# EStormLynn/Peter-Shirley-Ray-Tracing-the-next-week

Hardware: AMD Instinct MI355X
Metric: Msamples/s (pixels×spp/s) + achieved HBM GB/s, final() 500×500×1000spp (higher is better)
Workload: dtype f32

## Files before the change

### include/rt_hip.h

```cpp
#ifndef RT_HIP_H
#define RT_HIP_H
#include <stdint.h>

#ifdef __cplusplus
extern "C" {
#endif

#define RT_ABI_VERSION 2

typedef enum rt_status {
    RT_OK = 0,
    RT_ERR_INVALID = -1,
    RT_ERR_HIP = -2,
    RT_ERR_NOMEM = -3,
    RT_ERR_UNSUPPORTED = -4
} rt_status;

enum rt_prim_kind {
    RT_PRIM_SPHERE = 0,
    RT_PRIM_MOVING_SPHERE = 1,
    RT_PRIM_XY_RECT = 2,
    RT_PRIM_XZ_RECT = 3,
    RT_PRIM_YZ_RECT = 4
};

typedef struct rt_prim {
    int32_t kind;
    int32_t material;
    int32_t instance;
    int32_t flip;
    float p[12];
// ... 123 lines not shown
    double cycles_media;
    double cycles_shade;
    double grid;
    double wave_iterations;
    double wave_node_trips;
    double wave_prim_trips;
    double wave_sphere_draw_trips;
    double lane_sphere_draw_trips;
    double chunk;
    double batches;
    double lds_level;
    double stack_depth;
    double scan_groups;
    double prescan;
    double wave_exhaust_first_us;
    double wave_exhaust_last_us;
    double wave_end_first_us;
    double wave_end_mean_us;
    double wave_end_last_us;
    double wave_shade_passes;
    double wave_shade_kinds;
    double lane_scatters;
    double cycles_scatter;
} rt_stats;

typedef struct rt_scene rt_scene;

int rt_scene_create(const rt_scene_desc *d, int device, rt_scene **out);
void rt_scene_destroy(rt_scene *s);

int rt_render_tile(rt_scene *s, const rt_camera_desc *cam, const rt_render_params *p,
                   int x0, int y0, int w, int h, float *out_rgb, rt_stats *stats);

int rt_render_tiles(rt_scene *s, const rt_camera_desc *cam, const rt_render_params *p,
                    const int32_t *tiles, int ntiles, float *out_dev, void *stream, rt_stats *stats);

int rt_device_alloc(int device, uint64_t bytes, void **out);
int rt_device_free(void *ptr);
int rt_copy_to_host(void *dst, const void *src_dev, uint64_t bytes);
int rt_device_count(int *out);

int rt_math_probe(int fn, const float *a, const float *b, float *out, int64_t n);

#define RT_DIST_ID_BYTES 128
typedef struct rt_dist rt_dist;
int rt_dist_unique_id(uint8_t id[RT_DIST_ID_BYTES]);
// ... 45 lines not shown
```

### peter-shirley-ray-tracing-the-next-week_amd/csrc/hip/rt_device.h

```cpp
#pragma once
#include <hip/hip_runtime.h>
#include <stdint.h>
#include <type_traits>

#include "rt_layout.h"
#include "rt_libm.h"
#include "rt_log_table.h"
#include "rt_kernel.h"

#define RT_FLT_MAX 0x1.fffffep+127f
#ifndef RT_SHADE_LEAN
#define RT_SHADE_LEAN 117
#endif
#define RT_INF __builtin_huge_valf()

namespace {

__device__ __forceinline__ uint64_t wballot(bool b) { return __builtin_amdgcn_ballot_w64(b); }

struct V3 { float x, y, z; };
__device__ __forceinline__ V3 mk(float a, float b, float c) { V3 r; r.x = a; r.y = b; r.z = c; return r; }
__device__ __forceinline__ float unset_f() {
    float x;
    asm volatile("; unset %0" : "=v"(x));
    return x;
}
__device__ __forceinline__ V3 unset_v3() { return mk(unset_f(), unset_f(), unset_f()); }
__device__ __forceinline__ V3 add(V3 a, V3 b) { return mk(a.x + b.x, a.y + b.y, a.z + b.z); }
__device__ __forceinline__ V3 sub(V3 a, V3 b) { return mk(a.x - b.x, a.y - b.y, a.z - b.z); }
__device__ __forceinline__ V3 mul(V3 a, V3 b) { return mk(a.x * b.x, a.y * b.y, a.z * b.z); }
__device__ __forceinline__ V3 scale(float t, V3 v) { return mk(t * v.x, t * v.y, t * v.z); }
__device__ __forceinline__ V3 divs(V3 v, float t) { return mk(v.x / t, v.y / t, v.z / t); }
__device__ __forceinline__ V3 neg(V3 v) { return mk(-v.x, -v.y, -v.z); }
__device__ __forceinline__ float dot(V3 a, V3 b) { return a.x * b.x + a.y * b.y + a.z * b.z; }
__device__ __forceinline__ float len(V3 v) { return sqrtf(v.x * v.x + v.y * v.y + v.z * v.z); }
__device__ __forceinline__ V3 unit(V3 v) { return divs(v, len(v)); }
__device__ __forceinline__ float comp(V3 v, int i) { return i == 0 ? v.x : (i == 1 ? v.y : v.z); }

struct Ray { V3 o, d; float time; };

__device__ __forceinline__ float div_rn(float x, float b, float y) {
    const float q = x * y;
    return __builtin_fmaf(__builtin_fmaf(-q, b, x), y, q);
}
__device__ __forceinline__ V3 divs_rn(V3 v, float t, float y) { return mk(div_rn(v.x, t, y), div_rn(v.y, t, y), div_rn(v.z, t, y)); }
__device__ __forceinline__ bool normal_recip(float y) {
    const float m = __builtin_fabsf(y);
    return m >= 0x1p-126f && m <= 0x1.fffffep+127f;
}
struct Recip { float a, y; bool ok; };
__device__ __forceinline__ Recip recip_of(float a, bool use) {
    Recip r;
    r.a = a;
    r.y = 1.0f / a;
    r.ok = wballot(use && !normal_recip(r.y)) == 0ull;
    return r;
}
__device__ __forceinline__ float div_by(float x, const Recip &r) { return r.ok ? div_rn(x, r.a, r.y) : x / r.a; }
__device__ __forceinline__ V3 at(const Ray &r, float t) { return add(r.o, scale(t, r.d)); }

constexpr uint64_t kGamma = 0x9E3779B97F4A7C15ull;
constexpr uint64_t kLcgA = 0x5DEECE66Dull, kLcgC = 0xBull, kLcgM = 0xFFFFFFFFFFFFull;
__host__ __device__ __forceinline__ uint64_t mix64(uint64_t z) {
    z = (z ^ (z >> 30)) * 0xBF58476D1CE4E5B9ull;
    z = (z ^ (z >> 27)) * 0x94D049BB133111EBull;
    return z ^ (z >> 31);
}
__device__ __forceinline__ double u48(uint64_t z) {
    const uint64_t bits = 0x3FF0000000000000ull | ((z >> 12) & 0x000FFFFFFFFFFFF0ull);
    return __longlong_as_double((long long)bits) - 1.0;
}
__device__ __forceinline__ double u48x(uint64_t x) {
    return __longlong_as_double((long long)(0x3FF0000000000000ull | (x << 4))) - 1.0;
}
__device__ __forceinline__ uint64_t lcg_step(uint64_t x) {
    const uint32_t xl = (uint32_t)x, xh = (uint32_t)(x >> 32);
    static_assert(kLcgC == 11, "the drand48 increment is the inline constant of v_mad_u64_u32 below");
    uint64_t p, cy;
    uint32_t hi;
    asm("v_mad_u64_u32 %0, %1, %2, %3, 11" : "=v"(p), "=s"(cy) : "v"(xl), "s"(0xDEECE66Du));
    asm("v_mad_u32_u16 %0, %1, 5, %2" : "=v"(hi) : "v"(xl), "v"((uint32_t)(p >> 32)));
    asm("v_mad_u32_u16 %0, %1, %2, %3" : "=v"(hi) : "v"(xh), "s"(0xE66Du), "v"(hi));
    return ((uint64_t)(hi & 0xFFFFu) << 32) | (uint32_t)p;
}
typedef unsigned U4j __attribute__((ext_vector_type(4)));
__device__ __forceinline__ uint64_t lcg_jump(uint64_t x, U4j jt) {
    const uint32_t xl = (uint32_t)x, xh = (uint32_t)(x >> 32);
    const uint64_t c = ((uint64_t)jt.w << 32) | jt.z;
    uint64_t p, cy;
    uint32_t hi;
    asm("v_mad_u64_u32 %0, %1, %2, %3, %4" : "=v"(p), "=s"(cy) : "v"(xl), "v"(jt.x), "v"(c));
    asm("v_mad_u32_u16 %0, %1, %2, %3" : "=v"(hi) : "v"(xl), "v"(jt.y), "v"((uint32_t)(p >> 32)));
    asm("v_mad_u32_u16 %0, %1, %2, %3" : "=v"(hi) : "v"(xh), "v"(jt.x), "v"(hi));
    return ((uint64_t)(hi & 0xFFFFu) << 32) | (uint32_t)p;
}
#define RT_LCG_JUMPS 193
// ... 258 lines not shown
            float oi, di, oj, dj;
            if (kind == RT_PRIM_XY_RECT) { oi = r.o.x; di = r.d.x; oj = r.o.y; dj = r.d.y; }
            else if (kind == RT_PRIM_XZ_RECT) { oi = r.o.x; di = r.d.x; oj = r.o.z; dj = r.d.z; }
            else { oi = r.o.y; di = r.d.y; oj = r.o.z; dj = r.d.z; }
            const float a = oi + t * di, b = oj + t * dj;
            h.u = (a - g0.x) / (g0.y - g0.x);
            h.v = (b - g0.z) / (g0.w - g0.z);
        }
    }
    if (flip) h.n = neg(h.n);
    if (kInst && inst >= 0) to_world(insts, inst, h.p, h.n);
    return h;
}

__device__ __forceinline__ uint32_t lanes_below(uint64_t mask);
__device__ __forceinline__ bool first_active() { return lanes_below(wballot(1)) == 0; }

struct Counters {
    uint64_t samples = 0, segments = 0, nodes = 0, spheres = 0, mspheres = 0, rects = 0, instanced = 0, media = 0,
             shades = 0, noise = 0;
    uint64_t w_iters = 0, w_nodes = 0, w_prims = 0, w_rius = 0, l_rius = 0;
    uint64_t w_shade = 0, w_kinds = 0, l_scatter = 0;
    uint64_t ball[RT_BALL_N] = {0, 0, 0, 0, 0, 0, 0, 0};
    __device__ __forceinline__ void prim(int kind) {
        const int k = kind & 0xff;
        if (k == RT_PRIM_SPHERE) spheres++;
        else if (k == RT_PRIM_MOVING_SPHERE) mspheres++;
        else rects++;
        if (kind & 0x100) instanced++;
    }
};

template <bool kCount, bool kInst = true>
__device__ __forceinline__ float boundary_t(const float4 *B, const float4 *insts, int first, int count, const Ray &r,
                                            float tmin, Counters &cnt) {
    float best = RT_INF;
    for (int q = 0; q < count; ++q) {
        int key, kind;
        float t = prim_t<kInst>(B, insts, (uint32_t)(first + q), r, tmin, key, kind);
        if (kCount) cnt.prim(kind);
        if (t < best) best = t;
    }
    return best;
}

template <class RV, class PM>
// ... 626 lines not shown
}

typedef LogConsts MediaConsts;
typedef __attribute__((address_space(3))) const volatile MediaConsts LdsMediaConsts;
struct MediumRec {
    int4 md;
    float4 g0;
    float4 mm;
};
#ifndef RT_LDS_MEDIA
#define RT_LDS_MEDIA 8
#endif
template <int kBlock>
__device__ __forceinline__ void load_media(const RtKernelArgs &A, MediumRec *lds) {
    const int n = min(A.nmedia, RT_LDS_MEDIA);
    for (int i = threadIdx.x; i < n; i += kBlock) {
        const int4 md = A.media[i];
        lds[i].md = md;
        lds[i].g0 = A.bprims[md.x * 4 + 0];
        lds[i].mm = A.bprims[md.x * 4 + 1];
    }
}

template <bool kCount, bool kInst = true>
__device__ __forceinline__ void medium_one(const RtKernelArgs &A, const MediumRec &M, int k, const Ray &r, const Recip &rd,
                                           const Recip &ra, uint64_t xk, bool &have, float &best_t,
                                           int &med_mat, LdsMediaConsts *mc, Counters &cnt) {
    const float dlen = rd.a;
    if (kCount) cnt.media++;
    const int4 md = M.md;
    float r1, r2;
    bool ok;
    const float4 bm = M.mm;
    if (md.y == 1 && (fbits(bm.x) & 0xff) == RT_PRIM_SPHERE && fbits(bm.z) < 0) {
        if (kCount) cnt.spheres++;
        const float4 sg = M.g0;
        V3 oc = sub(r.o, mk(sg.x, sg.y, sg.z));
        const float a = ra.a;
        float b = dot(oc, r.d);
        float cc = dot(oc, oc) - sg.w * sg.w;
        float disc = b * b - a * cc;
        const bool valid = disc > 0;
        if (wballot(valid) == 0ull) return;
        const float sq = sqrtf(disc);
        const float ta = div_by(-b - sq, ra);
        const float tb = div_by(-b + sq, ra);
        const bool fa = ta < RT_FLT_MAX && ta > -RT_FLT_MAX, fb = tb < RT_FLT_MAX && tb > -RT_FLT_MAX;
        r1 = fa ? ta : tb;
        const float tmin2 = (float)((double)r1 + 0.0001);
        const bool ga = ta < RT_FLT_MAX && ta > tmin2, gb = tb < RT_FLT_MAX && tb > tmin2;
        r2 = ga ? ta : tb;
        ok = valid && (fa || fb) && (ga || gb);
    } else {
        r1 = boundary_t<kCount, kInst>(A.bprims, A.insts, md.x, md.y, r, -RT_FLT_MAX, cnt);
        ok = r1 != RT_INF;
        if (wballot(ok) == 0ull) return;
        r2 = boundary_t<kCount, kInst>(A.bprims, A.insts, md.x, md.y, r, (float)((double)r1 + 0.0001), cnt);
        ok = ok && r2 != RT_INF;
    }
    const float tmax = have ? best_t : RT_FLT_MAX;
    r1 = r1 < A.tmin ? A.tmin : r1;
    r2 = r2 > tmax ? tmax : r2;
    ok = ok && !(r1 >= r2);
    if (wballot(ok) == 0ull) return;
    r1 = r1 < 0 ? 0.f : r1;
    const float distance_inside_boundary = (r2 - r1) * dlen;
    const float neg_inv_density = __int_as_float(md.z);
#if !defined(__HIP_DEVICE_COMPILE__)
    const LogConsts lc{mc->c07, mc->c06, mc->c02, mc->c025, mc->c03};
#else
    uint32_t mca = (uint32_t)(size_t)mc;
    asm volatile("" : "+v"(mca));
    const LogConsts lc = *(__attribute__((address_space(3))) const LogConsts *)(size_t)mca;
#endif
    const float hit_distance = (float)((double)neg_inv_density * log_f64(u48x(xk), lc));
    const bool hit = ok && hit_distance < distance_inside_boundary;
    const float tm = r1 + div_by(hit_distance, rd);
    best_t = hit ? tm : best_t;
    have = have || hit;
    med_mat = hit ? md.w : med_mat;
}

template <bool kCount, bool kInst = true>
__device__ __forceinline__ int media_hit(const RtKernelArgs &A, const MediumRec *lds_media, LdsMediaConsts *mc, const Ray &r,
                                         const Recip &rd, Rng &g, bool &have, float &best_t, Counters &cnt) {
    const Recip ra = recip_of(dot(r.d, r.d), true);
    typedef unsigned U4v __attribute__((ext_vector_type(4)));
    typedef __attribute__((address_space(3))) const U4v LdsU4;
    int med_mat = -1;
    const int nl = min(A.nmedia, RT_LDS_MEDIA);
    for (int k = 0; k < nl; ++k) {
        const LdsU4 *p = (const LdsU4 *)lds_media + 3 * k;
        const U4v x = p[0], y = p[1], z = p[2];
        MediumRec M;
        M.md = make_int4((int)x.x, (int)x.y, (int)x.z, (int)x.w);
        M.g0 = make_float4(__uint_as_float(y.x), __uint_as_float(y.y), __uint_as_float(y.z), __uint_as_float(y.w));
        M.mm = make_float4(__uint_as_float(z.x), __uint_as_float(z.y), __uint_as_float(z.z), __uint_as_float(z.w));
        g.xm = lcg_step(g.xm);
        medium_one<kCount, kInst>(A, M, k, r, rd, ra, g.xm, have, best_t, med_mat, mc, cnt);
    }
    for (int k = RT_LDS_MEDIA; k < A.nmedia; ++k) {
        MediumRec M;
        M.md = A.media[k];
        M.g0 = A.bprims[M.md.x * 4 + 0];
        M.mm = A.bprims[M.md.x * 4 + 1];
        g.xm = lcg_step(g.xm);
        medium_one<kCount, kInst>(A, M, k, r, rd, ra, g.xm, have, best_t, med_mat, mc, cnt);
    }
    return med_mat;
}

struct ShadeOut {
    bool scattered;
    V3 att, emitted;
    Ray ray;
};

struct ShadeState {
    int kind;
    bool live;
    bool wants_sphere;
    V3 tv;
};

template <bool kCount, bool kUV = true, bool kChecker = true, class RV = const float4 *, class PM = const int *>
__device__ __forceinline__ ShadeState shade_begin(const RtKernelArgs &A, bool ready, bool have, const Hit &hr, int depth,
                                                  CoopSlot *slots, uint32_t lane, Counters &cnt, RV ranvec, PM perm) {
    const bool shading = ready && have;
    ShadeState st;
    st.kind = -1;
    st.live = false;
// ... 124 lines not shown
```

### peter-shirley-ray-tracing-the-next-week_amd/csrc/hip/rt_kernel.h

```cpp
#pragma once
#include <hip/hip_runtime.h>
#include <stdint.h>

#define RT_BLOCK 256

#define RT_LDS_BLOCK 1024
#define RT_LDS_NODE_CAP 1024
#define RT_LDS_NODE_BYTES (4 * RT_LDS_NODE_CAP * 16)
#define RT_LDS_NODE_BYTES_MEDIA (14 * RT_LDS_NODE_CAP * 4)
#define RT_LDS_STACK_BYTES(depth) ((RT_LDS_BLOCK / 64) * (depth) * 64 * 2)
#define RT_LDS_MAX_PRIMS 4096
#define RT_LDS_BUDGET 163840

#define RT_FEAT_INST 1
#define RT_FEAT_UV 2
#define RT_FEAT_CHECKER 4
#define RT_FEAT_PRESCAN 8
#define RT_FEAT_MEDIA 16
#define RT_FEAT_ALL 31

#define RT_WAVE_LOG_WORDS 12

struct RtKernelArgs {
    const float4 *nodes;
// ... 6 lines not shown
    const float4 *ranvec;
    const int *perm;
    const uint8_t *texels;
    uint32_t root;
    uint32_t nnodes;
    int bvh_width;
    int has_bvh;
    int nmedia;
    int features;
    int need_dlen;
    const float4 *groups;
    int ngroups;
    int scan;
    uint32_t nprims;
    int nprescan;
    int cell_first, cell_n;
    float cell_c[3], cell_r2;
    float cell_rin2;
    int ball_waves;
    int ball_batch;
    int ball_claim;
    int ball_park;
    int ball_drain;
    int lds_nodes;
    int stack_depth;
    float org[3], llc[3], hor[3], ver[3], cu[3], cv[3];
    float lens, ct0, ct1;
    int nx, ny, ns, max_depth;
    float rnx, rny;
    float tmin;
    int background;
    int chunk, nchunks;
    uint32_t sample_offset;
    uint64_t seed;
    const uint32_t *job_xy;
    uint32_t npix;
    uint32_t nitems;
    uint32_t ndeep;
    uint32_t ndeep_items;
    uint32_t claim;
    uint32_t nbig;
    uint32_t claim_tail;
    float *slab;
    uint32_t *counter;
    unsigned long long *stats;
    unsigned long long *wave_log;
// ... 16 lines not shown
```

### peter-shirley-ray-tracing-the-next-week_amd/csrc/hip/rt_kernel.hip

```cpp
#include <algorithm>
#include <atomic>
#include <type_traits>

#include "rt_device.h"

namespace {


#define RT_SLAB_FLOATS 3
#ifndef RT_READY_BATCH
#define RT_READY_BATCH 48
#endif

#ifndef RT_DESCEND_STEPS
#define RT_DESCEND_STEPS 2
#endif


#ifndef RT_DRY_LANES
#define RT_DRY_LANES 16
#endif


#define RT_PRE 64
// ... 507 lines not shown
                            if (wballot(ra || rb) == 0ull) test_pair(std::integral_constant<int, 1>());
                            else if (wballot(!ra || sb) == 0ull) test_pair(std::integral_constant<int, 2>());
                            else test_pair(std::integral_constant<int, 3>());
                        }
                    }
                    if (node == RT_EMPTY_CHILD) phase = PH_READY;
                }
            }
        }
        mark(1);
        const bool ready = phase == PH_READY;

        bool have = false;
        const float dlen = (ready && A.need_dlen) ? len(r.d) : 0.f;
        const Recip rd = recip_of(dlen, ready && A.need_dlen);
        Hit hr;
        if (RT_SHADE_LEAN & 2) {
            hr.p = unset_v3(); hr.n = unset_v3(); hr.u = unset_f(); hr.v = unset_f(); hr.mat = 0;
        } else {
            hr.p = mk(0, 0, 0); hr.n = mk(0, 0, 0); hr.u = 0.f; hr.v = 0.f; hr.mat = 0;
        }
        if (ready) {
            have = best_prim != 0xFFFFFFFFu;
            const int med_mat = kMedia ? media_hit<kCount, kInst>(A, lds_media, (LdsMediaConsts *)&lds_mconst, r, rd, g, have,
                                                                  best_t, cnt)
                                       : -1;
            if (med_mat >= 0) {
                hr.p = at(r, best_t);
                hr.n = mk(1, 0, 0);
                hr.mat = med_mat;
            } else if (have) {
                hr = prim_record<kInst, kUV>(A.prims, A.insts, A.mats, best_prim, r, best_t);
            }
        }

        mark(2);
        typedef __attribute__((address_space(3))) const F4v LdsRanvec;
        typedef __attribute__((address_space(3))) const int LdsPerm;
        const ShadeState st = kBall ? shade_begin<kCount, kUV, kChecker>(A, ready, have, hr, depth, slots, lane, cnt,
                                                                         (LdsRanvec *)lds_ranvec, (LdsPerm *)lds_perm)
                                    : shade_begin<kCount, kUV, kChecker>(A, ready, have, hr, depth, slots, lane, cnt,
                                                                         A.ranvec, A.perm);
        const bool ends = shade_ends(ready, have, st);
        if (kCount) {
            const bool sc = ready && !ends;
            if (wballot(sc) != 0ull) {
                const int kinds = (wballot(sc && st.kind == RT_MAT_LAMBERTIAN) != 0ull) +
                                  (wballot(sc && st.kind == RT_MAT_METAL) != 0ull) +
                                  (wballot(sc && st.kind == RT_MAT_DIELECTRIC) != 0ull) +
// ... 67 lines not shown
            const uint32_t hw = __builtin_amdgcn_s_getreg((31 << 11) | 4);
            const uint32_t xcc = __builtin_amdgcn_s_getreg((15 << 11) | 20);
            unsigned long long *W = A.wave_log + RT_WAVE_LOG_WORDS * ((size_t)blockIdx.x * (kBlock / 64) + wave);
            W[0] = rt_start;
            W[1] = rt_exhaust ? rt_exhaust : rt_end;
            W[2] = rt_end;
            W[3] = ((unsigned long long)xcc << 32) | hw;
            W[4] = rt_items;
            W[5] = dr_iters;
            W[6] = dr_live;
            W[7] = dr_taken;
            for (int k = 0; k < 4; ++k) W[8 + k] = dr_prof[k];
        }
    }
    if (kCount) {
        uint64_t w[8] = {cnt.w_iters, cnt.w_nodes, cnt.w_prims, cnt.w_rius, cnt.l_rius, cnt.w_shade, cnt.w_kinds, cnt.l_scatter};
        for (int k = 0; k < 8; ++k) {
            uint64_t x = w[k];
            for (int off = 32; off > 0; off >>= 1) x += __shfl_down(x, off);
            if (lane == 0 && x) atomicAdd(&A.stats[k < 5 ? RT_STAT_WAVE + k : RT_STAT_SHADE + (k - 5)], (unsigned long long)x);
        }
    }

    if (kCount && kBall && lane == 0)
        for (int k = 0; k < RT_BALL_N; ++k)
            if (cnt.ball[k]) atomicAdd(&A.stats[RT_STAT_BALL + k], (unsigned long long)cnt.ball[k]);
    if (kCount) {
        uint64_t v[RT_CNT_N] = {cnt.samples, cnt.segments, cnt.nodes, cnt.spheres, cnt.mspheres, cnt.rects,
                                cnt.instanced, cnt.media, cnt.shades, cnt.noise};
        for (int k = 0; k < RT_CNT_N; ++k) {
            uint64_t x = v[k];
            for (int off = 32; off > 0; off >>= 1) x += __shfl_down(x, off);
            if (lane == 0 && x) atomicAdd(&A.stats[k], (unsigned long long)x);
        }
    }
}

#undef A

__global__ __launch_bounds__(256) void rt_resolve(const float *__restrict__ slab, uint32_t npix, int nchunks, float k,
                                                  float4 *__restrict__ acc, int mode,
                                                  const uint32_t *__restrict__ out_index, float *__restrict__ out) {
    uint32_t p = blockIdx.x * blockDim.x + threadIdx.x;
    if (p >= npix) return;
    const uint32_t o = out_index[p];
    V3 col = mk(0, 0, 0);
// ... 178 lines not shown
```

### peter-shirley-ray-tracing-the-next-week_amd/csrc/host/capi.cpp

```cpp
#include <hip/hip_runtime.h>

#include <algorithm>
#include <chrono>
#include <cmath>
#include <cstdio>
#include <cstring>
#include <map>
#include <mutex>
#include <stdexcept>
#include <string>
#include <vector>

#include "rt_hip.h"
#include "../rt_layout.h"
#include "../hip/rt_kernel.h"
#include "bvh.h"
#include "rtnw.h"

namespace {

thread_local std::string g_err;

int fail(int code, const std::string &msg) {
    g_err = msg;
// ... 90 lines not shown
           20.0 * items;
}

}

int rt_internal_fail(int code, const std::string &msg) { return fail(code, msg); }

struct rt_scene {
    int device = 0;
    int cus = 0;
    int grid[3] = {0, 0, 0};
    bool lds_nodes = false;
    int stack_depth = 0;
    hipStream_t own_stream = nullptr;
    void *arena = nullptr;
    void *nodes = nullptr, *prims = nullptr, *bprims = nullptr, *media = nullptr, *mats = nullptr, *texs = nullptr,
         *insts = nullptr, *ranvec = nullptr, *perm = nullptr, *texels = nullptr, *groups = nullptr;
    bool scan = false;
    int nprescan = 0;
    int cell_first = 0, cell_n = 0;
    float cell_c[3] = {0, 0, 0}, cell_r2 = 0, cell_rin2 = 0;
    int ngroups = 0;
    uint32_t root = 0;
    int has_bvh = 0, nmedia = 0, bvh_depth = 0, nnodes = 0, nprims = 0, bvh_width = 2, ninstances = 0;
    bool has_moving = false;
    bool has_uv = false;
    bool has_checker = false;
    bool has_specular = false;
    float time0 = 0, time1 = 1;
    std::vector<int32_t> job_tiles;
    uint32_t job_ndeep = 0;
    std::vector<float> deep_balls;
    uint32_t npix = 0;
    void *job_xy = nullptr, *job_out = nullptr;
    void *slab = nullptr;
    size_t slab_bytes = 0;
    void *acc = nullptr;
    size_t acc_bytes = 0;
    void *counter = nullptr, *stats = nullptr;
    void *host_out = nullptr;
    size_t host_out_bytes = 0;
    hipEvent_t ev[3] = {nullptr, nullptr, nullptr};
};

static int scene_features(const rt_scene *s) {
    if (const char *e = std::getenv("RTNW_FEAT_ALL"))
// ... 388 lines not shown
    stage(arena, &s->prims, prims);
    stage(arena, &s->bprims, bprims);
    stage(arena, &s->media, media);
    stage(arena, &s->mats, mats);
    stage(arena, &s->texs, texs);
    stage(arena, &s->insts, insts);
    stage(arena, &s->groups, groups);
    stage(arena, &s->ranvec, ranvec);
    stage(arena, &s->perm, perm);
    stage(arena, &s->texels, texels);
    trace("device records");
    if (int rc = commit(arena, &s->arena)) return cleanup(rc);
    trace("upload (one allocation)");
    s->root = bvh.root;
    s->has_bvh = d->nprims > 0;
    s->nmedia = d->nmedia;
    for (int i = 0; i < d->nmedia; i++) {
        const rt_medium &m = d->media[i];
        if (m.boundary_count != 1 || !(m.density > 0)) continue;
        const rt_prim &bp = d->boundary_prims[m.boundary_first];
        const float R = std::fabs(bp.p[3]);
        if (bp.kind != RT_PRIM_SPHERE || bp.instance >= 0 || !(1.0f / m.density < 0.5f * R)) continue;
        s->deep_balls.insert(s->deep_balls.end(), {bp.p[0], bp.p[1], bp.p[2], R});
    }
    s->bvh_depth = bvh.depth;
    s->nnodes = (int)bvh.node_count();
    s->bvh_width = bvh.width;
    s->nprims = d->nprims;
    s->ninstances = d->ninstances;
    s->ngroups = (int)groups.size();
    s->nprescan = s->scan ? 0 : (int)big.size();

    if ((e = hipDeviceGetAttribute(&s->cus, hipDeviceAttributeMultiprocessorCount, device)) != hipSuccess)
        return cleanup(hip_fail(e, "hipDeviceGetAttribute"));
    for (int mode = 0; mode < 3; mode++) {
        int bpc = 0;
        if ((e = occupancy(&bpc, mode, s->scan ? 0 : s->bvh_width)) != hipSuccess)
            return cleanup(hip_fail(e, "occupancy query"));
        if (const char *e = std::getenv("RTNW_BLOCKS_PER_CU")) bpc = std::min(bpc, std::max(1, std::atoi(e)));
        s->grid[mode] = std::max(1, bpc) * s->cus;
    }
    {
        s->stack_depth = s->bvh_depth + 1;
        const long need_actual = rt_lds_need_bytes(scene_features(s), s->stack_depth);
        bool want = true;
        if (const char *e = std::getenv("RTNW_LDS_BVH")) want = std::atoi(e) != 0;
// ... 193 lines not shown
    a.ball_park = env_int("RTNW_BALL_PARK", 1, 0, 1);
    a.ball_drain = env_int("RTNW_BALL_DRAIN", 1, 0, 1);
    a.nprims = (uint32_t)s->nprims;
    a.stack_depth = s->stack_depth;
    a.features = scene_features(s);
    for (int k = 0; k < 3; k++) {
        a.org[k] = cam->origin[k];
        a.llc[k] = cam->lower_left_corner[k];
        a.hor[k] = cam->horizontal[k];
        a.ver[k] = cam->vertical[k];
        a.cu[k] = cam->u[k];
        a.cv[k] = cam->v[k];
    }
    a.lens = cam->lens_radius;
    a.ct0 = cam->time0;
    a.ct1 = cam->time1;
    a.nx = p->nx;
    a.ny = p->ny;
    a.rnx = 1.0f / (float)p->nx;
    a.rny = 1.0f / (float)p->ny;
    a.ns = p->spp;
    a.max_depth = p->max_depth;
    a.tmin = p->t_min;
    a.background = p->background;
    a.chunk = chunk;
    a.seed = p->seed;
    a.job_xy = (const uint32_t *)s->job_xy;
    a.npix = s->npix;
    a.slab = (float *)s->slab;
    a.counter = (uint32_t *)s->counter;
    a.stats = (unsigned long long *)s->stats;
    const char *wave_log_path = prof ? std::getenv("RTNW_WAVE_LOG") : nullptr;
    unsigned long long *wave_log = nullptr;
    struct FreeOnExit {
        unsigned long long *&p;
        ~FreeOnExit() { if (p) (void)hipFree(p); }
    } wave_log_guard{wave_log};
    const size_t wave_log_n = (size_t)s->grid[2] * ((s->lds_nodes ? RT_LDS_BLOCK : RT_BLOCK) / 64) * RT_WAVE_LOG_WORDS;
    if (wave_log_path) {
        HIP_TRY(hipMalloc(&wave_log, wave_log_n * sizeof(unsigned long long)));
        HIP_TRY(hipMemsetAsync(wave_log, 0, wave_log_n * sizeof(unsigned long long), stream));
    }
    a.wave_log = wave_log;

    const uint32_t ns_total = sum_in ? p->sample_offset + (uint32_t)p->spp : (uint32_t)p->spp;
    const float k = (float)(1.0 / (double)(float)ns_total);
// ... 61 lines not shown
            stats->samples = (double)c[RT_CNT_SAMPLES];
            stats->segments = (double)c[RT_CNT_SEGMENTS];
            stats->node_visits = (double)c[RT_CNT_NODES];
            stats->sphere_tests = (double)c[RT_CNT_SPHERES];
            stats->moving_sphere_tests = (double)c[RT_CNT_MSPHERES];
            stats->rect_tests = (double)c[RT_CNT_RECTS];
            stats->instanced_tests = (double)c[RT_CNT_INSTANCED];
            stats->medium_tests = (double)c[RT_CNT_MEDIA];
            stats->shades = (double)c[RT_CNT_SHADES];
            stats->noise_evals = (double)c[RT_CNT_NOISE];
            stats->algorithmic_bytes = algorithmic_bytes(*stats, (double)s->npix * (double)nchunks_total, s->bvh_width);
            unsigned long long w[5];
            HIP_TRY(hipMemcpy(w, (unsigned long long *)s->stats + RT_STAT_WAVE, sizeof w, hipMemcpyDeviceToHost));
            stats->wave_iterations = (double)w[0];
            stats->wave_node_trips = (double)w[1];
            stats->wave_prim_trips = (double)w[2];
            stats->wave_sphere_draw_trips = (double)w[3];
            stats->lane_sphere_draw_trips = (double)w[4];
            unsigned long long sh[3];
            HIP_TRY(hipMemcpy(sh, (unsigned long long *)s->stats + RT_STAT_SHADE, sizeof sh, hipMemcpyDeviceToHost));
            stats->wave_shade_passes = (double)sh[0];
            stats->wave_shade_kinds = (double)sh[1];
            stats->lane_scatters = (double)sh[2];
            if (std::getenv("RTNW_TRACE")) {
                unsigned long long b[RT_BALL_N];
                HIP_TRY(hipMemcpy(b, (unsigned long long *)s->stats + RT_STAT_BALL, sizeof b, hipMemcpyDeviceToHost));
                std::fprintf(stderr,
                             "rtnw ball waves: iterations %llu, live lanes / iteration %.1f, traversal rounds / iteration %.2f, "
                             "cell-decided segments in ball waves %llu, pushes refused (pool full) %llu (of %.0f segments), pushed in %llu, "
                             "pushed out %llu, taken %llu\n",
                             b[RT_BALL_ITERS], b[RT_BALL_ITERS] ? (double)b[RT_BALL_LIVE] / b[RT_BALL_ITERS] : 0.0,
                             b[RT_BALL_ITERS] ? (double)b[RT_BALL_ROUNDS] / b[RT_BALL_ITERS] : 0.0, b[RT_BALL_CELL_BALL],
                             b[RT_BALL_DENIED], stats->segments, b[RT_BALL_PUSH_IN], b[RT_BALL_PUSH_OUT], b[RT_BALL_TAKEN]);
            }
        }
        if (prof) {
            unsigned long long c[RT_STATS_LEN];
            HIP_TRY(hipMemcpy(c, s->stats, sizeof c, hipMemcpyDeviceToHost));
            if (std::getenv("RTNW_TRACE")) {
                const unsigned long long *b = c + RT_STAT_BALL;
                std::fprintf(stderr,
                             "rtnw ball waves (profile): iterations %llu of %llu; cycles claim %llu of %llu, traverse %llu of "
                             "%llu, media %llu of %llu, shade %llu of %llu\n",
                             b[4], b[5], b[0], c[RT_STAT_PROF], b[1], c[RT_STAT_PROF + 1], b[2], c[RT_STAT_PROF + 2], b[3],
                             c[RT_STAT_PROF + 3]);
            }
// ... 159 lines not shown
```

### peter-shirley-ray-tracing-the-next-week_amd/csrc/rt_layout.h

```cpp
#pragma once
#include <stdint.h>

#include "rt_hip.h"

#define RT_STACK_DEPTH 24
#define RT_STACK_DEPTH_W8 32
#define RT_MAX_BVH_DEPTH 23
#define RT_MAX_LEAF 8
#define RT_MAX_INSTANCE_OPS 6
#define RT_MAX_CHECKER_DEPTH 16

#define RT_LEAF_BIT 0x80000000u
#define RT_EMPTY_CHILD 0xFFFFFFFFu
#define RT_LEAF_REF(first, count) (RT_LEAF_BIT | ((uint32_t)((count) - 1) << 24) | (uint32_t)(first))
#define RT_LEAF_FIRST(ref) ((ref) & 0x00FFFFFFu)
#define RT_LEAF_COUNT(ref) ((((ref) >> 24) & 0x7Fu) + 1)

struct rt_dnode2 {
    float b[3][4];
    uint32_t ch[4];
};

struct rt_dnode4 {
    float q[6][4];
// ... 43 lines not shown
    float scale;
    float color[3];
    int32_t pad;
};

struct rt_dinstance {
    int32_t nops, pad[3];
    float ops[RT_MAX_INSTANCE_OPS][4];
};

struct rt_dmedium {
    int32_t first, count;
    float neg_inv_density;
    int32_t material;
};

enum {
    RT_CNT_SAMPLES = 0, RT_CNT_SEGMENTS, RT_CNT_NODES, RT_CNT_SPHERES, RT_CNT_MSPHERES, RT_CNT_RECTS,
    RT_CNT_INSTANCED, RT_CNT_MEDIA, RT_CNT_SHADES, RT_CNT_NOISE, RT_CNT_N
};
enum {
    RT_STAT_PROF = RT_CNT_N, RT_STAT_WAVE = RT_CNT_N + 4, RT_STAT_TIME = RT_CNT_N + 9, RT_STAT_SHADE = RT_CNT_N + 16,
    RT_STAT_BALL = RT_CNT_N + 20,
    RT_STATS_LEN = RT_CNT_N + 28
};
enum { RT_BALL_ITERS = 0, RT_BALL_LIVE, RT_BALL_ROUNDS, RT_BALL_CELL_BALL, RT_BALL_DENIED, RT_BALL_PUSH_IN,
       RT_BALL_PUSH_OUT, RT_BALL_TAKEN, RT_BALL_N };
```

### peter-shirley-ray-tracing-the-next-week_amd/rtnw.py

```python
from __future__ import annotations

import ctypes
import os
import re

import numpy as np

HERE = os.path.dirname(os.path.abspath(__file__))
LIB_PATH = os.environ.get("RTNW_LIB") or os.path.join(HERE, "librt_hip.so")
HEADER = os.path.join(os.path.dirname(HERE), "include", "rt_hip.h")

RT_OK = 0
RT_BG_BLACK, RT_BG_SKY = 0, 1
RT_FLAG_COUNT = 1
RT_FLAG_PROFILE = 2
RT_FLAG_SUM_IN = 4
RT_FLAG_SUM_OUT = 8
RT_CHECKPOINT_MAGIC = 0x4B435452


class RtError(RuntimeError):
    def __init__(self, code, msg):
        super().__init__(f"rt_hip error {code}: {msg}")
        self.code = code
# ... 36 lines not shown

class RtCameraDesc(ctypes.Structure):
    _fields_ = [("origin", ctypes.c_float * 3), ("lower_left_corner", ctypes.c_float * 3),
                ("horizontal", ctypes.c_float * 3), ("vertical", ctypes.c_float * 3), ("u", ctypes.c_float * 3),
                ("v", ctypes.c_float * 3), ("w", ctypes.c_float * 3), ("lens_radius", ctypes.c_float),
                ("time0", ctypes.c_float), ("time1", ctypes.c_float)]


class RtRenderParams(ctypes.Structure):
    _fields_ = [("nx", ctypes.c_int32), ("ny", ctypes.c_int32), ("spp", ctypes.c_int32), ("max_depth", ctypes.c_int32),
                ("t_min", ctypes.c_float), ("background", ctypes.c_int32), ("chunk", ctypes.c_int32),
                ("flags", ctypes.c_int32), ("sample_offset", ctypes.c_uint32), ("pad", ctypes.c_uint32),
                ("seed", ctypes.c_uint64)]


class RtStats(ctypes.Structure):
    _fields_ = [(n, ctypes.c_double) for n in (
        "samples", "segments", "node_visits", "sphere_tests", "moving_sphere_tests", "rect_tests", "instanced_tests",
        "medium_tests", "shades", "noise_evals", "algorithmic_bytes", "kernel_ms", "resolve_ms",
        "cycles_claim", "cycles_traverse", "cycles_media", "cycles_shade", "grid", "wave_iterations",
        "wave_node_trips", "wave_prim_trips", "wave_sphere_draw_trips", "lane_sphere_draw_trips", "chunk",
        "batches", "lds_level", "stack_depth", "scan_groups", "prescan", "wave_exhaust_first_us",
        "wave_exhaust_last_us", "wave_end_first_us", "wave_end_mean_us", "wave_end_last_us",
        "wave_shade_passes", "wave_shade_kinds", "lane_scatters", "cycles_scatter")]

    def as_dict(self):
        return {n: getattr(self, n) for n, _ in self._fields_}


class RtCheckpoint(ctypes.Structure):
    _fields_ = [("magic", ctypes.c_uint32), ("version", ctypes.c_uint32), ("nx", ctypes.c_int32),
                ("ny", ctypes.c_int32), ("samples_done", ctypes.c_uint32), ("max_depth", ctypes.c_int32),
                ("background", ctypes.c_int32), ("t_min", ctypes.c_float), ("seed", ctypes.c_uint64),
                ("job_hash", ctypes.c_uint64), ("count", ctypes.c_uint64)]


_lib = None


def lib():
    global _lib
    if _lib is None:
        try:
            import torch
        except Exception:
            pass
        if not os.path.exists(LIB_PATH):
            raise RuntimeError(f"{LIB_PATH} is missing: build it with `make -C {HERE}` (no CPU fallback exists)")
        L = ctypes.CDLL(LIB_PATH)
        P = ctypes.POINTER
# ... 373 lines not shown
```

Measured before the change: 5086.

## Add cooperative sphere-media path with conservative early exclusion of media tests

When every participating medium is bounded by a single non-instanced sphere, a new path pre-screens each medium. It uses a conservative lower bound on the free-flight distance drawn from the per-medium RNG stream, and a conservative geometric test for miss, behind, or beyond the current hit. Only media that survive the screening get the full root, clip and log evaluation, one per lane per wave pass, with lcg_jump used to recover each medium's random state. This is meant to avoid the costly log and division work for media that cannot produce a hit, while keeping results identical. In exchange it adds ballot loops and jump-table lookups, and if the bounds are wrong the output could drift. New media statistics counters and an ABI bump come along with it.

```diff
diff --git a/include/rt_hip.h b/include/rt_hip.h
--- a/include/rt_hip.h
+++ b/include/rt_hip.h
@@ -6,7 +6,7 @@
 extern "C" {
 #endif
 
-#define RT_ABI_VERSION 2
+#define RT_ABI_VERSION 3
 
 typedef enum rt_status {
     RT_OK = 0,
@@ -176,6 +176,11 @@
     double wave_shade_kinds;
     double lane_scatters;
     double cycles_scatter;
+    double media_iterations;
+    double media_pending_iterations;
+    double media_passes;
+    double media_rounds;
+    double media_lanes[8];
 } rt_stats;
 
 typedef struct rt_scene rt_scene;
diff --git a/peter-shirley-ray-tracing-the-next-week_amd/csrc/hip/rt_device.h b/peter-shirley-ray-tracing-the-next-week_amd/csrc/hip/rt_device.h
--- a/peter-shirley-ray-tracing-the-next-week_amd/csrc/hip/rt_device.h
+++ b/peter-shirley-ray-tracing-the-next-week_amd/csrc/hip/rt_device.h
@@ -19,7 +19,7 @@
 __device__ __forceinline__ uint64_t wballot(bool b) { return __builtin_amdgcn_ballot_w64(b); }
 
 struct V3 { float x, y, z; };
-__device__ __forceinline__ V3 mk(float a, float b, float c) { V3 r; r.x = a; r.y = b; r.z = c; return r; }
+__host__ __device__ __forceinline__ V3 mk(float a, float b, float c) { V3 r; r.x = a; r.y = b; r.z = c; return r; }
 __device__ __forceinline__ float unset_f() {
     float x;
     asm volatile("; unset %0" : "=v"(x));
@@ -27,24 +27,24 @@
 }
 __device__ __forceinline__ V3 unset_v3() { return mk(unset_f(), unset_f(), unset_f()); }
 __device__ __forceinline__ V3 add(V3 a, V3 b) { return mk(a.x + b.x, a.y + b.y, a.z + b.z); }
-__device__ __forceinline__ V3 sub(V3 a, V3 b) { return mk(a.x - b.x, a.y - b.y, a.z - b.z); }
+__host__ __device__ __forceinline__ V3 sub(V3 a, V3 b) { return mk(a.x - b.x, a.y - b.y, a.z - b.z); }
 __device__ __forceinline__ V3 mul(V3 a, V3 b) { return mk(a.x * b.x, a.y * b.y, a.z * b.z); }
 __device__ __forceinline__ V3 scale(float t, V3 v) { return mk(t * v.x, t * v.y, t * v.z); }
 __device__ __forceinline__ V3 divs(V3 v, float t) { return mk(v.x / t, v.y / t, v.z / t); }
 __device__ __forceinline__ V3 neg(V3 v) { return mk(-v.x, -v.y, -v.z); }
-__device__ __forceinline__ float dot(V3 a, V3 b) { return a.x * b.x + a.y * b.y + a.z * b.z; }
+__host__ __device__ __forceinline__ float dot(V3 a, V3 b) { return a.x * b.x + a.y * b.y + a.z * b.z; }
 __device__ __forceinline__ float len(V3 v) { return sqrtf(v.x * v.x + v.y * v.y + v.z * v.z); }
 __device__ __forceinline__ V3 unit(V3 v) { return divs(v, len(v)); }
 __device__ __forceinline__ float comp(V3 v, int i) { return i == 0 ? v.x : (i == 1 ? v.y : v.z); }
 
 struct Ray { V3 o, d; float time; };
 
-__device__ __forceinline__ float div_rn(float x, float b, float y) {
+__host__ __device__ __forceinline__ float div_rn(float x, float b, float y) {
     const float q = x * y;
     return __builtin_fmaf(__builtin_fmaf(-q, b, x), y, q);
 }
 __device__ __forceinline__ V3 divs_rn(V3 v, float t, float y) { return mk(div_rn(v.x, t, y), div_rn(v.y, t, y), div_rn(v.z, t, y)); }
-__device__ __forceinline__ bool normal_recip(float y) {
+__host__ __device__ __forceinline__ bool normal_recip(float y) {
     const float m = __builtin_fabsf(y);
     return m >= 0x1p-126f && m <= 0x1.fffffep+127f;
 }
@@ -56,7 +56,7 @@
     r.ok = wballot(use && !normal_recip(r.y)) == 0ull;
     return r;
 }
-__device__ __forceinline__ float div_by(float x, const Recip &r) { return r.ok ? div_rn(x, r.a, r.y) : x / r.a; }
+__host__ __device__ __forceinline__ float div_by(float x, const Recip &r) { return r.ok ? div_rn(x, r.a, r.y) : x / r.a; }
 __device__ __forceinline__ V3 at(const Ray &r, float t) { return add(r.o, scale(t, r.d)); }
 
 constexpr uint64_t kGamma = 0x9E3779B97F4A7C15ull;
@@ -70,8 +70,8 @@
     const uint64_t bits = 0x3FF0000000000000ull | ((z >> 12) & 0x000FFFFFFFFFFFF0ull);
     return __longlong_as_double((long long)bits) - 1.0;
 }
-__device__ __forceinline__ double u48x(uint64_t x) {
-    return __longlong_as_double((long long)(0x3FF0000000000000ull | (x << 4))) - 1.0;
+__host__ __device__ __forceinline__ double u48x(uint64_t x) {
+    return __builtin_bit_cast(double, 0x3FF0000000000000ull | (x << 4)) - 1.0;
 }
 __device__ __forceinline__ uint64_t lcg_step(uint64_t x) {
     const uint32_t xl = (uint32_t)x, xh = (uint32_t)(x >> 32);
@@ -376,6 +376,8 @@
     uint64_t w_iters = 0, w_nodes = 0, w_prims = 0, w_rius = 0, l_rius = 0;
     uint64_t w_shade = 0, w_kinds = 0, l_scatter = 0;
     uint64_t ball[RT_BALL_N] = {0, 0, 0, 0, 0, 0, 0, 0};
+    uint64_t m_iters = 0, m_pending = 0, m_passes = 0, m_rounds = 0;
+    uint64_t m_lanes[8] = {0, 0, 0, 0, 0, 0, 0, 0};
     __device__ __forceinline__ void prim(int kind) {
         const int k = kind & 0xff;
         if (k == RT_PRIM_SPHERE) spheres++;
@@ -1048,6 +1050,85 @@
     }
 }
 
+__device__ __forceinline__ LogConsts media_consts(LdsMediaConsts *mc) {
+#if !defined(__HIP_DEVICE_COMPILE__)
+    return LogConsts{mc->c07, mc->c06, mc->c02, mc->c025, mc->c03};
+#else
+    uint32_t mca = (uint32_t)(size_t)mc;
+    asm volatile("" : "+v"(mca));
+    return *(__attribute__((address_space(3))) const LogConsts *)(size_t)mca;
+#endif
+}
+
+struct MedQuad { float b, cc, disc; };
+__host__ __device__ __forceinline__ MedQuad med_quad(const Ray &r, float a, float4 sg) {
+    const V3 oc = sub(r.o, mk(sg.x, sg.y, sg.z));
+    MedQuad q;
+    q.b = dot(oc, r.d);
+    q.cc = dot(oc, oc) - sg.w * sg.w;
+    q.disc = q.b * q.b - a * q.cc;
+    return q;
+}
+struct MedSpan { float r1, r2; bool ok; };
+__host__ __device__ __forceinline__ MedSpan med_roots(float b, float disc, const Recip &ra) {
+    const bool valid = disc > 0;
+    const float sq = sqrtf(disc);
+    const float ta = div_by(-b - sq, ra);
+    const float tb = div_by(-b + sq, ra);
+    const bool fa = ta < RT_FLT_MAX && ta > -RT_FLT_MAX, fb = tb < RT_FLT_MAX && tb > -RT_FLT_MAX;
+    MedSpan m;
+    m.r1 = fa ? ta : tb;
+    const float tmin2 = (float)((double)m.r1 + 0.0001);
+    const bool ga = ta < RT_FLT_MAX && ta > tmin2, gb = tb < RT_FLT_MAX && tb > tmin2;
+    m.r2 = ga ? ta : tb;
+    m.ok = valid && (fa || fb) && (ga || gb);
+    return m;
+}
+__host__ __device__ __forceinline__ void med_clip(MedSpan &m, float tmin, bool have, float best_t) {
+    const float tmax = have ? best_t : RT_FLT_MAX;
+    m.r1 = m.r1 < tmin ? tmin : m.r1;
+    m.r2 = m.r2 > tmax ? tmax : m.r2;
+    m.ok = m.ok && !(m.r1 >= m.r2);
+}
+__host__ __device__ __forceinline__ bool med_flight(const MedSpan &m, float dlen, const Recip &rd, float neg_inv_density,
+                                                    uint64_t xk, const LogConsts &lc, float &tm) {
+    const float r1 = m.r1 < 0 ? 0.f : m.r1;
+    const float distance_inside_boundary = (m.r2 - r1) * dlen;
+    const float hit_distance = (float)((double)neg_inv_density * log_f64(u48x(xk), lc));
+    tm = r1 + div_by(hit_distance, rd);
+    return m.ok && hit_distance < distance_inside_boundary;
+}
+__host__ __device__ __forceinline__ bool med_sphere_lane(const Ray &r, const Recip &ra, const Recip &rd, float4 sg,
+                                                         float neg_inv_density, float tmin, bool have, float best_t,
+                                                         uint64_t xk, const LogConsts &lc, float &tm) {
+    const MedQuad q = med_quad(r, ra.a, sg);
+    MedSpan m = med_roots(q.b, q.disc, ra);
+    med_clip(m, tmin, have, best_t);
+    return med_flight(m, rd.a, rd, neg_inv_density, xk, lc, tm);
+}
+
+__host__ __device__ __forceinline__ bool med_excl_flight(uint64_t xk, float neg_inv_density, float dub) {
+    const double w = 2.0 - __builtin_bit_cast(double, 0x3FF0000000000000ull | (xk << 4));
+    const double lb = w * (-(double)neg_inv_density * (1.0 - 0x1p-19));
+    return lb >= (double)dub;
+}
+__host__ __device__ __forceinline__ bool med_excl_geo(const MedQuad &q, const Recip &ra, bool have, float best_t) {
+    const bool miss = !(q.disc > 0);
+    const bool behind = q.cc > 0 && q.b >= 0x1p-60f;
+#if defined(__HIP_DEVICE_COMPILE__)
+    const float sa = __builtin_amdgcn_sqrtf(q.disc);
+#else
+    const float sa = sqrtf(q.disc);
+#endif
+    const float s = sa * (1.0f + 0x1p-20f);
+    const float n = (-q.b - s) - (__builtin_fabsf(q.b) + s) * 0x1p-20f;
+    const float e = n * ra.y;
+    const float el = e - __builtin_fabsf(e) * 0x1p-20f;
+    const float bar = best_t > 0x1p-100f ? best_t : 0x1p-100f;
+    const bool beyond = have && normal_recip(ra.y) && el >= bar;
+    return miss || behind || beyond;
+}
+
 template <bool kCount, bool kInst = true>
 __device__ __forceinline__ void medium_one(const RtKernelArgs &A, const MediumRec &M, int k, const Ray &r, const Recip &rd,
                                            const Recip &ra, uint64_t xk, bool &have, float &best_t,
@@ -1055,53 +1136,27 @@
     const float dlen = rd.a;
     if (kCount) cnt.media++;
     const int4 md = M.md;
-    float r1, r2;
-    bool ok;
+    MedSpan m;
     const float4 bm = M.mm;
     if (md.y == 1 && (fbits(bm.x) & 0xff) == RT_PRIM_SPHERE && fbits(bm.z) < 0) {
         if (kCount) cnt.spheres++;
-        const float4 sg = M.g0;
-        V3 oc = sub(r.o, mk(sg.x, sg.y, sg.z));
-        const float a = ra.a;
-        float b = dot(oc, r.d);
-        float cc = dot(oc, oc) - sg.w * sg.w;
-        float disc = b * b - a * cc;
-        const bool valid = disc > 0;
-        if (wballot(valid) == 0ull) return;
-        const float sq = sqrtf(disc);
-        const float ta = div_by(-b - sq, ra);
-        const float tb = div_by(-b + sq, ra);
-        const bool fa = ta < RT_FLT_MAX && ta > -RT_FLT_MAX, fb = tb < RT_FLT_MAX && tb > -RT_FLT_MAX;
-        r1 = fa ? ta : tb;
-        const float tmin2 = (float)((double)r1 + 0.0001);
-        const bool ga = ta < RT_FLT_MAX && ta > tmin2, gb = tb < RT_FLT_MAX && tb > tmin2;
-        r2 = ga ? ta : tb;
-        ok = valid && (fa || fb) && (ga || gb);
+        const MedQuad q = med_quad(r, ra.a, M.g0);
+        if (wballot(q.disc > 0) == 0ull) return;
+        m = med_roots(q.b, q.disc, ra);
     } else {
-        r1 = boundary_t<kCount, kInst>(A.bprims, A.insts, md.x, md.y, r, -RT_FLT_MAX, cnt);
-        ok = r1 != RT_INF;
-        if (wballot(ok) == 0ull) return;
-        r2 = boundary_t<kCount, kInst>(A.bprims, A.insts, md.x, md.y, r, (float)((double)r1 + 0.0001), cnt);
-        ok = ok && r2 != RT_INF;
-    }
-    const float tmax = have ? best_t : RT_FLT_MAX;
-    r1 = r1 < A.tmin ? A.tmin : r1;
-    r2 = r2 > tmax ? tmax : r2;
-    ok = ok && !(r1 >= r2);
-    if (wballot(ok) == 0ull) return;
-    r1 = r1 < 0 ? 0.f : r1;
-    const float distance_inside_boundary = (r2 - r1) * dlen;
-    const float neg_inv_density = __int_as_float(md.z);
-#if !defined(__HIP_DEVICE_COMPILE__)
-    const LogConsts lc{mc->c07, mc->c06, mc->c02, mc->c025, mc->c03};
-#else
-    uint32_t mca = (uint32_t)(size_t)mc;
-    asm volatile("" : "+v"(mca));
-    const LogConsts lc = *(__attribute__((address_space(3))) const LogConsts *)(size_t)mca;
-#endif
-    const float hit_distance = (float)((double)neg_inv_density * log_f64(u48x(xk), lc));
-    const bool hit = ok && hit_distance < distance_inside_boundary;
-    const float tm = r1 + div_by(hit_distance, rd);
+        m.r1 = boundary_t<kCount, kInst>(A.bprims, A.insts, md.x, md.y, r, -RT_FLT_MAX, cnt);
+        m.ok = m.r1 != RT_INF;
+        if (wballot(m.ok) == 0ull) return;
+        m.r2 = boundary_t<kCount, kInst>(A.bprims, A.insts, md.x, md.y, r, (float)((double)m.r1 + 0.0001), cnt);
+        m.ok = m.ok && m.r2 != RT_INF;
+    }
+    med_clip(m, A.tmin, have, best_t);
+    if (wballot(m.ok) == 0ull) return;
+    if (kCount && first_active()) cnt.m_passes++;
+    if (kCount && m.ok && k < 8) cnt.m_lanes[k]++;
+    const LogConsts lc = media_consts(mc);
+    float tm;
+    const bool hit = med_flight(m, dlen, rd, __int_as_float(md.z), xk, lc, tm);
     best_t = hit ? tm : best_t;
     have = have || hit;
     med_mat = hit ? md.w : med_mat;
@@ -1114,6 +1169,7 @@
     typedef unsigned U4v __attribute__((ext_vector_type(4)));
     typedef __attribute__((address_space(3))) const U4v LdsU4;
     int med_mat = -1;
+    if (kCount && first_active()) cnt.m_iters++;
     const int nl = min(A.nmedia, RT_LDS_MEDIA);
     for (int k = 0; k < nl; ++k) {
         const LdsU4 *p = (const LdsU4 *)lds_media + 3 * k;
@@ -1133,6 +1189,90 @@
         g.xm = lcg_step(g.xm);
         medium_one<kCount, kInst>(A, M, k, r, rd, ra, g.xm, have, best_t, med_mat, mc, cnt);
     }
+    return med_mat;
+}
+
+template <bool kCount>
+__device__ __forceinline__ int media_hit_coop(const RtKernelArgs &A, const MediumRec *lds_media, LdsMediaConsts *mc,
+                                              const LdsJump *jt, const Ray &r, const Recip &rd, Rng &g, bool &have,
+                                              float &best_t, Counters &cnt) {
+    typedef unsigned U4v __attribute__((ext_vector_type(4)));
+    typedef unsigned U2v __attribute__((ext_vector_type(2)));
+    typedef __attribute__((address_space(3))) const U4v LdsU4;
+    typedef __attribute__((address_space(3))) const U2v LdsU2;
+    static_assert(sizeof(MediumRec) == 48, "the record reads below: md.zw at dword 2, g0 at dword 4 of 12");
+    static_assert((RT_LDS_MEDIA & (RT_LDS_MEDIA - 1)) == 0 && RT_LDS_MEDIA <= 32, "a lane's pending mask and its index clamp");
+    const LdsU4 *rec4 = (const LdsU4 *)lds_media;
+    const LdsU2 *rec2 = (const LdsU2 *)lds_media;
+    const Recip ra = recip_of(dot(r.d, r.d), true);
+    const float dlen = rd.a;
+    const int n = min(A.nmedia, RT_LDS_MEDIA);
+    const uint64_t xm0 = g.xm;
+    uint32_t pend = 0;
+    {
+        const float dub = have ? best_t * dlen : RT_INF;
+        uint64_t x = xm0;
+        for (int k = 0; k < n; ++k) {
+            x = lcg_step(x);
+            pend |= med_excl_flight(x, __uint_as_float(rec2[6 * k + 1].x), dub) ? 0u : 1u << k;
+        }
+    }
+    if (kCount) {
+        cnt.media += (uint64_t)n;
+        cnt.spheres += (uint64_t)n;
+        if (first_active()) cnt.m_iters++;
+        if (wballot(pend != 0u) != 0ull && first_active()) cnt.m_pending++;
+    }
+    int med_mat = -1;
+    while (wballot(pend != 0u) != 0ull) {
+        int k = -1;
+        float qb = 0.f, qd = 0.f;
+        bool open = pend != 0u;
+        do {
+            const int kk = (__builtin_ffs((int)pend) - 1) & (RT_LDS_MEDIA - 1);
+            const U4v gv = rec4[3 * kk + 1];
+            const MedQuad q = med_quad(r, ra.a, make_float4(__uint_as_float(gv.x), __uint_as_float(gv.y),
+                                                            __uint_as_float(gv.z), __uint_as_float(gv.w)));
+            const bool ex = med_excl_geo(q, ra, have, best_t);
+            if (kCount && first_active()) cnt.m_rounds++;
+            if (open) {
+                if (ex) {
+                    pend &= pend - 1u;
+                } else {
+                    k = kk;
+                    qb = q.b;
+                    qd = q.disc;
+                }
+                open = ex && pend != 0u;
+            }
+        } while (wballot(open) != 0ull);
+        const bool on = k >= 0;
+        if (wballot(on) == 0ull) break;
+        const int kc = on ? k : 0;
+        const U2v zw = rec2[6 * kc + 1];
+        const uint64_t xk = lcg_jump(xm0, jt[kc + 1]);
+        MedSpan m = med_roots(qb, qd, ra);
+        med_clip(m, A.tmin, have, best_t);
+        m.ok = m.ok && on;
+        if (kCount) {
+            if (first_active()) cnt.m_passes++;
+            for (int j = 0; j < 8; ++j) cnt.m_lanes[j] += (m.ok && k == j) ? 1u : 0u;
+        }
+        pend &= on ? ~(1u << k) : ~0u;
+        const LogConsts lc = media_consts(mc);
+        float tm;
+        const bool hit = med_flight(m, dlen, rd, __uint_as_float(zw.x), xk, lc, tm);
+        best_t = hit ? tm : best_t;
+        have = have || hit;
+        med_mat = hit ? (int)zw.y : med_mat;
+        {
+            const int kn = (__builtin_ffs((int)pend) - 1) & (RT_LDS_MEDIA - 1);
+            const bool ex = med_excl_flight(lcg_jump(xm0, jt[kn + 1]), __uint_as_float(rec2[6 * kn + 1].x),
+                                            have ? best_t * dlen : RT_INF);
+            pend &= ex ? pend - 1u : ~0u;
+        }
+    }
+    g.xm = lcg_jump(xm0, jt[n]);
     return med_mat;
 }
 
diff --git a/peter-shirley-ray-tracing-the-next-week_amd/csrc/hip/rt_kernel.h b/peter-shirley-ray-tracing-the-next-week_amd/csrc/hip/rt_kernel.h
--- a/peter-shirley-ray-tracing-the-next-week_amd/csrc/hip/rt_kernel.h
+++ b/peter-shirley-ray-tracing-the-next-week_amd/csrc/hip/rt_kernel.h
@@ -52,6 +52,7 @@
     int ball_claim;
     int ball_park;
     int ball_drain;
+    int media_coop;
     int lds_nodes;
     int stack_depth;
     float org[3], llc[3], hor[3], ver[3], cu[3], cv[3];
diff --git a/peter-shirley-ray-tracing-the-next-week_amd/csrc/hip/rt_kernel.hip b/peter-shirley-ray-tracing-the-next-week_amd/csrc/hip/rt_kernel.hip
--- a/peter-shirley-ray-tracing-the-next-week_amd/csrc/hip/rt_kernel.hip
+++ b/peter-shirley-ray-tracing-the-next-week_amd/csrc/hip/rt_kernel.hip
@@ -553,9 +553,11 @@
         }
         if (ready) {
             have = best_prim != 0xFFFFFFFFu;
-            const int med_mat = kMedia ? media_hit<kCount, kInst>(A, lds_media, (LdsMediaConsts *)&lds_mconst, r, rd, g, have,
-                                                                  best_t, cnt)
-                                       : -1;
+            int med_mat = -1;
+            if (kMedia && (kInst || !A.media_coop || A.nmedia > RT_LDS_MEDIA))
+                med_mat = media_hit<kCount, kInst>(A, lds_media, (LdsMediaConsts *)&lds_mconst, r, rd, g, have, best_t, cnt);
+            else if (kMedia)
+                med_mat = media_hit_coop<kCount>(A, lds_media, (LdsMediaConsts *)&lds_mconst, jt, r, rd, g, have, best_t, cnt);
             if (med_mat >= 0) {
                 hr.p = at(r, best_t);
                 hr.n = mk(1, 0, 0);
@@ -669,6 +671,15 @@
         }
     }
 
+    if (kCount && kMedia) {
+        uint64_t w[RT_MEDIA_N] = {cnt.m_iters, cnt.m_pending, cnt.m_passes, cnt.m_rounds, cnt.m_lanes[0], cnt.m_lanes[1],
+                                  cnt.m_lanes[2], cnt.m_lanes[3], cnt.m_lanes[4], cnt.m_lanes[5], cnt.m_lanes[6], cnt.m_lanes[7]};
+        for (int k = 0; k < RT_MEDIA_N; ++k) {
+            uint64_t x = w[k];
+            for (int off = 32; off > 0; off >>= 1) x += __shfl_down(x, off);
+            if (lane == 0 && x) atomicAdd(&A.stats[RT_STAT_MEDIA + k], (unsigned long long)x);
+        }
+    }
     if (kCount && kBall && lane == 0)
         for (int k = 0; k < RT_BALL_N; ++k)
             if (cnt.ball[k]) atomicAdd(&A.stats[RT_STAT_BALL + k], (unsigned long long)cnt.ball[k]);
diff --git a/peter-shirley-ray-tracing-the-next-week_amd/csrc/host/capi.cpp b/peter-shirley-ray-tracing-the-next-week_amd/csrc/host/capi.cpp
--- a/peter-shirley-ray-tracing-the-next-week_amd/csrc/host/capi.cpp
+++ b/peter-shirley-ray-tracing-the-next-week_amd/csrc/host/capi.cpp
@@ -136,6 +136,7 @@
     float cell_c[3] = {0, 0, 0}, cell_r2 = 0, cell_rin2 = 0;
     int ngroups = 0;
     uint32_t root = 0;
+    bool sphere_media = false;
     int has_bvh = 0, nmedia = 0, bvh_depth = 0, nnodes = 0, nprims = 0, bvh_width = 2, ninstances = 0;
     bool has_moving = false;
     bool has_uv = false;
@@ -570,6 +571,13 @@
         const float R = std::fabs(bp.p[3]);
         if (bp.kind != RT_PRIM_SPHERE || bp.instance >= 0 || !(1.0f / m.density < 0.5f * R)) continue;
         s->deep_balls.insert(s->deep_balls.end(), {bp.p[0], bp.p[1], bp.p[2], R});
+    }
+    s->sphere_media = d->nmedia > 0;
+    for (int i = 0; i < d->nmedia; i++) {
+        const rt_medium &m = d->media[i];
+        if (m.boundary_count != 1) { s->sphere_media = false; break; }
+        const rt_prim &bp = d->boundary_prims[m.boundary_first];
+        if (bp.kind != RT_PRIM_SPHERE || bp.instance >= 0) { s->sphere_media = false; break; }
     }
     s->bvh_depth = bvh.depth;
     s->nnodes = (int)bvh.node_count();
@@ -809,6 +817,7 @@
     a.ns = p->spp;
     a.max_depth = p->max_depth;
     a.tmin = p->t_min;
+    a.media_coop = s->sphere_media && p->t_min >= 0 && env_int("RTNW_MEDIA_COOP", 1, 0, 1);
     a.background = p->background;
     a.chunk = chunk;
     a.seed = p->seed;
@@ -916,6 +925,13 @@
             stats->wave_shade_passes = (double)sh[0];
             stats->wave_shade_kinds = (double)sh[1];
             stats->lane_scatters = (double)sh[2];
+            unsigned long long md[RT_MEDIA_N];
+            HIP_TRY(hipMemcpy(md, (unsigned long long *)s->stats + RT_STAT_MEDIA, sizeof md, hipMemcpyDeviceToHost));
+            stats->media_iterations = (double)md[RT_MEDIA_ITERS];
+            stats->media_pending_iterations = (double)md[RT_MEDIA_PENDING];
+            stats->media_passes = (double)md[RT_MEDIA_PASSES];
+            stats->media_rounds = (double)md[RT_MEDIA_ROUNDS];
+            for (int k = 0; k < 8; k++) stats->media_lanes[k] = (double)md[RT_MEDIA_LANES + k];
             if (std::getenv("RTNW_TRACE")) {
                 unsigned long long b[RT_BALL_N];
                 HIP_TRY(hipMemcpy(b, (unsigned long long *)s->stats + RT_STAT_BALL, sizeof b, hipMemcpyDeviceToHost));
diff --git a/peter-shirley-ray-tracing-the-next-week_amd/csrc/rt_layout.h b/peter-shirley-ray-tracing-the-next-week_amd/csrc/rt_layout.h
--- a/peter-shirley-ray-tracing-the-next-week_amd/csrc/rt_layout.h
+++ b/peter-shirley-ray-tracing-the-next-week_amd/csrc/rt_layout.h
@@ -89,7 +89,9 @@
 enum {
     RT_STAT_PROF = RT_CNT_N, RT_STAT_WAVE = RT_CNT_N + 4, RT_STAT_TIME = RT_CNT_N + 9, RT_STAT_SHADE = RT_CNT_N + 16,
     RT_STAT_BALL = RT_CNT_N + 20,
-    RT_STATS_LEN = RT_CNT_N + 28
+    RT_STAT_MEDIA = RT_CNT_N + 28,
+    RT_STATS_LEN = RT_CNT_N + 40
 };
+enum { RT_MEDIA_ITERS = 0, RT_MEDIA_PENDING, RT_MEDIA_PASSES, RT_MEDIA_ROUNDS, RT_MEDIA_LANES, RT_MEDIA_N = RT_MEDIA_LANES + 8 };
 enum { RT_BALL_ITERS = 0, RT_BALL_LIVE, RT_BALL_ROUNDS, RT_BALL_CELL_BALL, RT_BALL_DENIED, RT_BALL_PUSH_IN,
        RT_BALL_PUSH_OUT, RT_BALL_TAKEN, RT_BALL_N };
diff --git a/peter-shirley-ray-tracing-the-next-week_amd/rtnw.py b/peter-shirley-ray-tracing-the-next-week_amd/rtnw.py
--- a/peter-shirley-ray-tracing-the-next-week_amd/rtnw.py
+++ b/peter-shirley-ray-tracing-the-next-week_amd/rtnw.py
@@ -82,10 +82,12 @@
         "wave_node_trips", "wave_prim_trips", "wave_sphere_draw_trips", "lane_sphere_draw_trips", "chunk",
         "batches", "lds_level", "stack_depth", "scan_groups", "prescan", "wave_exhaust_first_us",
         "wave_exhaust_last_us", "wave_end_first_us", "wave_end_mean_us", "wave_end_last_us",
-        "wave_shade_passes", "wave_shade_kinds", "lane_scatters", "cycles_scatter")]
+        "wave_shade_passes", "wave_shade_kinds", "lane_scatters", "cycles_scatter",
+        "media_iterations", "media_pending_iterations", "media_passes", "media_rounds")] + [
+        ("media_lanes", ctypes.c_double * 8)]
 
     def as_dict(self):
-        return {n: getattr(self, n) for n, _ in self._fields_}
+        return {n: (list(getattr(self, n)) if n == "media_lanes" else getattr(self, n)) for n, _ in self._fields_}
 
 
 class RtCheckpoint(ctypes.Structure):
```

Measured after the change: 4859. -4.5%, worse.
